# mitchelldurbincs/GeneralsReinforcementLearning

Hardware: AMD Instinct MI355X
Metric: env steps/sec (whole node), 20x20 4P fog-on; state bit-exact vs the C restatement of the Go engine (the reference's own test vectors pass on both) (higher is better)
Workload: dtype int32

## Files before the change

### generalsreinforcementlearning_amd/_lib.py

```python
import ctypes as C
import os

_PKG = os.path.dirname(os.path.abspath(__file__))
_LIB = None


class GvecError(RuntimeError):
    def __init__(self, code, msg):
        super().__init__(f"gvec error {code}: {msg}")
        self.code = code


class Config(C.Structure):
    _fields_ = [("abi_version", C.c_int32), ("num_envs", C.c_int32), ("max_width", C.c_int32), ("max_height", C.c_int32),
                ("max_players", C.c_int32), ("device", C.c_int32), ("fog_of_war", C.c_int32), ("prod_general", C.c_int32),
                ("prod_city", C.c_int32), ("prod_normal", C.c_int32), ("normal_growth_interval", C.c_int32),
                ("auto_reset", C.c_int32), ("reserved", C.c_int32 * 4)]


STATE_FIELDS = ["army", "owner", "type", "visible", "listed", "changed", "vis_changed", "turn", "done", "winner", "width",
                "height", "players", "alive", "army_count", "tile_count", "general_idx"]


class StateView(C.Structure):
# ... 89 lines not shown
    "gvec_reset_generated": (_i32, [_vp, _u64, _vp, _vp, _vp]),
    "gvec_reset_go_seeded": (_i32, [_vp, _vp, _vp, _vp, _vp]),
    "gvec_build_board_pool": (_i32, [_vp, _i32, _u64, _vp, _vp, _vp]),
    "gvec_step": (_i32, [_vp, _vp, _vp, _vp, _i32]),
    "gvec_legal_mask": (_i32, [_vp, _vp, _i32]),
    "gvec_player_visibility": (_i32, [_vp, _i32, _vp, _vp, _i32]),
    "gvec_read_state": (_i32, [_vp, _i32, _i32, C.POINTER(StateView), _i32]),
    "gvec_write_state": (_i32, [_vp, _i32, _i32, C.POINTER(StateView), _i32]),
    "gvec_rollout": (_i32, [_vp, _i32, _u64, _i32, _i32, C.POINTER(RolloutStats)]),
    "gvec_rollout_range": (_i32, [_vp, _i32, _i32, _i32, _u64, _i32]),
    "gvec_set_agent_mix": (_i32, [_vp, _i32, _i32]),
    "gvec_agent_actions": (_i32, [_vp, _u64, _i32, _vp, _i32]),
    "gvec_bot_actions": (_i32, [_vp, C.c_uint32, _u64, _i32, _vp, _i32]),
    "gvec_counters": (_i32, [_vp, C.POINTER(RolloutStats)]),
    "gvec_step_traffic_bytes": (_i32, [_vp, C.POINTER(C.c_int64)]),
    "gvec_experience_begin": (_i32, [_vp]),
    "gvec_experience_begin_range": (_i32, [_vp, _i32, _i32]),
    "gvec_experience_rewards": (_i32, [_vp, _vp, _vp, _i32]),
    "gvec_experience_record_layout": (_i32, [_vp, C.POINTER(C.c_int32)]),
    "gvec_experience_record_bytes": (_i32, [_vp]),
    "gvec_experience_records": (_i32, [_vp, _vp, _i32, _i32, _i32, _i32, _vp]),
    "gvec_record_agent_actions": (_i32, [_vp, _i32]),
    "gvec_expand_experience_records": (_i32, [_i32, _vp, C.POINTER(C.c_int32), _vp, _i32, _vp, _vp, _vp, _vp]),
    "gvec_pool_collect": (_i32, [_i32, _vp, C.POINTER(CollectArgs)]),
    "gvec_pool_collect_scratch_bytes": (_u64, [_i32]),
    "gvec_per_tree_bytes": (_u64, [C.c_int64]),
    "gvec_per_tree_layout": (_i32, [C.c_int64, C.POINTER(C.c_int64)]),
    "gvec_per_init": (_i32, [_i32, _vp, _vp, C.c_int64]),
    "gvec_per_push": (_i32, [_i32, _vp, _vp, C.c_int64, _vp, _vp, C.c_int64]),
    "gvec_per_update": (_i32, [_i32, _vp, _vp, C.c_int64, _vp, _vp, C.c_int64, C.c_float, C.c_float]),
# ... 67 lines not shown
```

### generalsreinforcementlearning_amd/csrc/gvec_api.hip

```cpp
#include <cstdarg>
#include <cstdio>
#include <new>

#include "gvec_handle.hpp"

static thread_local char g_err[512] = "";
void set_err(const char* fmt, ...) {
  va_list ap;
  va_start(ap, fmt);
  vsnprintf(g_err, sizeof g_err, fmt, ap);
  va_end(ap);
}

int32_t DevBuf::in_stage() const {
  if (slot >= 0) return GVEC_OK;
  set_err("a call staged more than %d arguments through its handle", Stage::kSlots);
  return GVEC_E_INVALID;
}

hipError_t DevBuf::alloc(size_t bytes) {
  if (bytes < 16) bytes = 16;
  if (h->stage_cap[slot] < bytes) {
    if (h->stage_ptr[slot]) {
      hipError_t e = hipStreamSynchronize(h->stream);
// ... 143 lines not shown
  h->stride = cfg->max_width * cfg->max_height;
  h->maxp = cfg->max_players;
  if (!pick_variant(cfg->max_players, h->stride, &h->var)) {
    set_err("no kernel variant for %d players / %d tiles", cfg->max_players, h->stride);
    return false;
  }
  h->fd = (h->stride <= 32 * (2 * h->var.nslot - 1)) ? 2 * h->var.nslot - 1 : 2 * h->var.nslot;
  h->row_dw = (int)round_up((size_t)(3 * h->var.maxp + 13) * h->fd, 4);
  h->army_dw = h->var.nslot * 64;
  h->mask_bytes = 16 * h->fd;
  h->mask_dw = h->mask_bytes / 4;
  h->stream = nullptr;
  return true;
}

extern "C" {

int32_t gvec_abi_version(void) { return GVEC_ABI_VERSION; }
const char* gvec_last_error(void) { return g_err; }

int32_t gvec_config_default(gvec_config* cfg) {
  if (!cfg) return GVEC_E_INVALID;
  memset(cfg, 0, sizeof *cfg);
  cfg->abi_version = GVEC_ABI_VERSION;
  cfg->num_envs = 1;
  cfg->max_width = 20;
  cfg->max_height = 20;
  cfg->max_players = 2;
  cfg->device = 0;
  cfg->fog_of_war = 1;
// ... 168 lines not shown
  return GVEC_OK;
}
int32_t gvec_host_free(void* p) {
  if (!p) return GVEC_OK;
  HIPCHK(hipHostFree(p));
  return GVEC_OK;
}

int32_t gvec_num_envs(const gvec_handle* h) { return h ? h->cfg.num_envs : GVEC_E_INVALID; }
int32_t gvec_tile_stride(const gvec_handle* h) { return h ? h->stride : GVEC_E_INVALID; }
int32_t gvec_mask_bytes(const gvec_handle* h) { return h ? h->mask_bytes : GVEC_E_INVALID; }
int64_t gvec_state_bytes_per_env(const gvec_handle* h) {
  return h ? (int64_t)4 * (HDR_DW + h->row_dw + h->army_dw) : (int64_t)GVEC_E_INVALID;
}

int32_t gvec_read_buffer(gvec_handle* h, int32_t which, uint64_t byte_offset, uint64_t bytes, void* host_dst) {
  if (!h || !host_dst) return GVEC_E_INVALID;
  if (h->sharded()) return sharded::unsupported("gvec_read_buffer");
  const size_t B = (size_t)h->cfg.num_envs;
  size_t total = 0;
  const void* base = nullptr;
  switch (which) {
    case GVEC_BUF_HEADER: base = h->d_hdr; total = B * HDR_DW * 4; break;
    case GVEC_BUF_LEGAL: base = h->d_legal; total = B * h->maxp * h->mask_bytes; break;
    case GVEC_BUF_ACTIONS: base = h->d_actions; total = B * h->maxp * sizeof(gvec_action); break;
    case GVEC_BUF_ERR: base = h->d_err; total = B * 4; break;
    default:
      set_err("gvec_read_buffer: buffer %d is not one of header / legal masks / actions / err", which);
      return GVEC_E_INVALID;
  }
// ... 43 lines not shown
```

### generalsreinforcementlearning_amd/csrc/gvec_api_engine.hip

```cpp
#include "gvec_handle.hpp"

namespace sharded {

static int32_t reset(gvec_handle* h, const int32_t* env_ids, int32_t n, const int32_t* army, const int8_t* owner, const uint8_t* type,
                     const int32_t* width, const int32_t* height, const int32_t* players, int32_t mem) {
  RET_IF(host_only(mem, "gvec_reset"));
  const size_t st = (size_t)h->stride;
  if (!env_ids) {
    return fan_range(h, 0, n, [=](gvec_handle* c, int lb, int cnt, size_t skip) {
      return gvec_reset(c, nullptr, cnt, army + skip * st, owner + skip * st, type + skip * st, width + skip, height + skip, players + skip, GVEC_MEM_HOST);
    });
  }
  struct Part {
    std::vector<int32_t> ids, w, hh, p, army;
    std::vector<int8_t> owner;
    std::vector<uint8_t> type;
  };
  auto parts = std::make_shared<std::vector<Part>>(h->shards.size());
  for (int i = 0; i < n; ++i) {
    const int e = env_ids[i];
    if (e < 0 || e >= h->cfg.num_envs) return GVEC_E_RANGE;
    size_t k = 0;
    while (e >= h->shards[k]->begin + h->shards[k]->n) ++k;
    Part& P = (*parts)[k];
// ... 325 lines not shown
  HIPCHK(hipSetDevice(h->cfg.device));
  HIPCHK(hipMemsetAsync(h->d_counters, 0, 3 * sizeof(unsigned long long), h->stream));
  HIPCHK(launch_counter_sum(h->d_hdr, h->cfg.num_envs, h->d_counters, h->stream));
  unsigned long long c[3];
  HIPCHK(hipMemcpyAsync(c, h->d_counters, sizeof c, hipMemcpyDeviceToHost, h->stream));
  HIPCHK(hipStreamSynchronize(h->stream));
  out->env_steps = (int64_t)c[0];
  out->aborted_turns = (int64_t)c[1];
  out->games_finished = (int64_t)c[2];
  out->reserved = 0;
  return GVEC_OK;
}

int32_t gvec_step_traffic_bytes(const gvec_handle* h, int64_t* out4) {
  if (!h || !out4) return GVEC_E_INVALID;
  static_assert(Planes<4>::MUTABLE == 2 * 4 + 3 && Planes<4>::LST - Planes<4>::MUTABLE == 10 && Planes<4>::COUNT - Planes<4>::LST == 4,
                "gvec_step_traffic_bytes restates the plane block's partition");
  const int64_t fd = h->fd, mp = h->var.maxp;
  const int nslot = h->var.nslot;
  const bool odd = fd == 2 * nslot - 1;
  const int64_t hdr = HDR_DW * 4;
  const int64_t mut = (2 * mp + 3) * fd * 4;
  const int64_t cst = (lean_derive_ok(nslot) ? 6 : 10) * fd * 4;
  const int64_t lst = mp * fd * 4;
  const int64_t a16 = (int64_t)h->army_dw * 2, a32 = (int64_t)h->army_dw * 4;
  out4[0] = hdr + mut + cst + a16 - (lean_half_last(nslot, odd) ? 64 : 0);
  out4[1] = hdr + mut + lean_fold_dwords((int)(2 * mp + 3), (int)fd) * 4 + a16;
  out4[2] = (int64_t)h->maxp * h->mask_bytes;
  out4[3] = 2 * lst + 2 * a32;
  return GVEC_OK;
}

int32_t gvec_agent_actions(gvec_handle* h, uint64_t seed, int32_t invalid_permille, gvec_action* actions, int32_t mem) {
  if (!h || !actions) return GVEC_E_INVALID;
  if (h->sharded()) {
    const size_t mp = (size_t)h->maxp;
    return sharded::fan_host(h, mem, "gvec_agent_actions", [=](gvec_handle* c, int begin, int) {
      return gvec_agent_actions(c, seed, invalid_permille, actions + begin * mp, GVEC_MEM_HOST);
    });
  }
  HIPCHK(hipSetDevice(h->cfg.device));
  StepArgs a = base_args(h);
  set_agent_seed(&a, seed, invalid_permille);
  a.actions_out = (mem == GVEC_MEM_HOST) ? h->d_actions : actions;
// ... 44 lines not shown
```

### generalsreinforcementlearning_amd/csrc/gvec_device.hpp

```cpp
#pragma once
#include <hip/hip_runtime.h>
#include <stdint.h>

#include "../../include/generals_vec.h"

extern "C" __device__ int gvec_llvm_writelane(int value, int lane, int vdst_in) __asm("llvm.amdgcn.writelane.i32");

#ifndef GVEC_NT
#define GVEC_NT 14
#endif
#define GVEC_NT_MASK 2
#define GVEC_NT_PLANE 4
#define GVEC_NT_ARMY 8
#ifndef GVEC_SC1
#define GVEC_SC1 1
#endif

#ifndef GVEC_LEAN
#define GVEC_LEAN 7
#endif

namespace gvec {

constexpr bool lean_derive_ok(int nslot) { return (GVEC_LEAN & 1) != 0 && 2 * nslot < 64 / (nslot <= 7 ? 4 : 2); }
constexpr bool lean_half_last(int nslot, bool odd) { return (GVEC_LEAN & 2) != 0 && odd && (nslot & 1) != 0; }
constexpr int lean_fold_dwords(int mutable_planes, int fd) { return (GVEC_LEAN & 4) != 0 ? ((mutable_planes * fd + 3) & ~3) - mutable_planes * fd : 0; }

typedef uint32_t u32x4 __attribute__((ext_vector_type(4)));

template <typename T>
__device__ __forceinline__ T ld_stream(const T* p) {
  if constexpr ((GVEC_NT & 1) != 0) return __builtin_nontemporal_load(p);
  return *p;
}
__device__ __forceinline__ void st_through(uint32_t* p, uint32_t v) { asm volatile("global_store_dword %0, %1, off sc1 nt" : : "v"(p), "v"(v) : "memory"); }
__device__ __forceinline__ void st_through(uint16_t* p, uint16_t v) {
  asm volatile("global_store_short %0, %1, off sc1 nt" : : "v"(p), "v"((uint32_t)v) : "memory");
}
__device__ __forceinline__ void st_through(float* p, float v) { asm volatile("global_store_dword %0, %1, off sc1 nt" : : "v"(p), "v"(v) : "memory"); }
__device__ __forceinline__ void st_through(u32x4* p, u32x4 v) {
  asm volatile("global_store_dwordx4 %0, %1, off sc1 nt\n\ts_nop 1" : : "v"(p), "v"(v) : "memory");
// ... 18 lines not shown
  H_GIDX = 12,
  H_RECIPW = 20,
  H_CNT_STEPS = 21,
  H_CNT_ABORT = 22,
  H_CNT_DONE = 23
};
constexpr uint32_t HF_DONE = 1u, HF_FOG = 2u, HF_WIDE = 4u;
constexpr uint32_t HF_SETUP = 8u;
constexpr uint32_t HF_SYNC = 16u;
constexpr uint32_t HF_VSMALL = 32u;
constexpr uint32_t HF_LDIFF = 128u;
constexpr uint32_t HF_FEWSPECIAL = 64u;

template <int MAXP>
struct Planes {
  static constexpr int OWN = 0, VIS = MAXP, CHG = 2 * MAXP, VCH = 2 * MAXP + 1, GT1 = 2 * MAXP + 2,
                       GEN = 2 * MAXP + 3, CITY = 2 * MAXP + 4, MTN = 2 * MAXP + 5, VALID = 2 * MAXP + 6, NCOL0 = 2 * MAXP + 7,
                       NCOLL = 2 * MAXP + 8, OK = 2 * MAXP + 9 , LST = 2 * MAXP + 13,
                       COUNT = 3 * MAXP + 13, MUTABLE = 2 * MAXP + 3, SHARED = 13 ;
};

constexpr uint32_t KF_AGENT = 1u;
constexpr uint32_t KF_EMIT = 2u;
constexpr uint32_t KF_AUTORESET = 4u;
constexpr uint32_t KF_LMVALID = 16u;

struct StepArgs {
  uint32_t* hdr;
  uint32_t* rows;
  uint32_t* army16;
  int32_t* army32;
  const gvec_action* actions;
  gvec_action* actions_out;
  int32_t* err;
// ... 323 lines not shown
```

### generalsreinforcementlearning_amd/csrc/gvec_kernels.hip

```cpp
#include "gvec_dispatch.hpp"
#include "gvec_turn.hpp"

namespace gvec {

constexpr int step_waves(int maxp, int nslot) {
  const int ppr = (nslot <= 7) ? 4 : 2;
  const int nr = (maxp + ppr - 1) / ppr;
  const int state = 3 * nr + 13 + nr + nslot + 4 * nr;
  const int need = state + (state + 32 <= 62 ? 32 : 40);
  const int alloc = (need + 7) / 8 * 8;
  const int w = 512 / alloc;
  return w > 8 ? 8 : (w < 2 ? 2 : w);
}

template <int MAXP, int NSLOT, bool AGENT, bool ODD>
__global__ __launch_bounds__(64 * WAVES_PER_BLOCK, step_waves(MAXP, NSLOT)) void step_kernel(StepArgs A) {
  constexpr int FD = 2 * NSLOT - (ODD ? 1 : 0);
  constexpr int ROW_DW = (Planes<MAXP>::COUNT * FD + 3) / 4 * 4;
  __shared__ int32_t army_shadow[WAVES_PER_BLOCK][NSLOT * 64];
  using B = Turn<MAXP, NSLOT>;
  __shared__ uint32_t act_scratch[WAVES_PER_BLOCK][B::ACT_SCRATCH_DW];
  const int wave = (int)(threadIdx.x >> 6), lane = lane_id();
  const int env = uni((int)blockIdx.x * WAVES_PER_BLOCK + wave);
  if (env >= A.num_envs) return;
  bool force_redeal = false;
  if constexpr (!AGENT) {
    const uint32_t f0 = (uint32_t)uni((int)reinterpret_cast<const uint32_t*>(A.actions)[((size_t)env * A.pstride) * 2 + 1]);
    if (f0 & GVEC_ACT_SKIP_ENV) {
      if (A.err && lane == 0) A.err[env] = 0;
      return;
    }
    force_redeal = (f0 & GVEC_ACT_RESET_ENV) != 0u;
  }
  B b;
  b.larmy = army_shadow[wave];
  b.lscr = act_scratch[wave];
  const ArmyRef army_env = army_ref<NSLOT>(A.army16, A.army32, env);
  load_turn<true, lean_half_last(NSLOT, ODD)>(b, A.hdr + (size_t)env * HDR_DW, A.rows + (size_t)env * ROW_DW, army_env, FD, A.zeros);
  b.small = !(b.hflags & HF_WIDE);
  const bool emit = (A.flags & KF_EMIT) != 0u;
  uint32_t m[B::NR][4];
  uint32_t err = 0u;
  bool types_dirty = false, changed = true;
  const bool can_redeal = (A.flags & KF_AUTORESET) && A.pool_size > 0;
  if (AGENT && A.actions_out && (b.hflags & HF_DONE)) {
    if (lane < A.pstride) reinterpret_cast<uint2*>(A.actions_out)[(size_t)env * A.pstride + lane] = make_uint2(0u, 0u);
  }
  if (can_redeal && ((b.hflags & HF_DONE) || force_redeal)) {
    redeal<MAXP, NSLOT>(b, A, env, FD, ROW_DW);
    types_dirty = true;
  } else if (b.hflags & HF_DONE) {
    err = GVEC_ERR_GAME_OVER;
    changed = false;
// ... 14 lines not shown
      if (A.actions_out) {
        uint32_t alo, ahi;
        agent_words<MAXP, NSLOT>(b, mine, alo, ahi);
        if (lane < A.pstride) reinterpret_cast<uint2*>(A.actions_out)[(size_t)env * A.pstride + lane] = make_uint2(alo, ahi);
      }
    } else {
      uint32_t alo = 0u, ahi = 0u;
      if (lane < A.pstride) {
        const uint2 w = reinterpret_cast<const uint2*>(A.actions)[(size_t)env * A.pstride + lane];
        alo = w.x;
        ahi = w.y;
      }
      av = b.prevalidate(alo, ahi);
    }
    bool aborted;
    err = b.turn_step(av, A, aborted);
    if (!(GVEC_PROFILE_SKIP & 32)) b.refresh_gt1();
    if (GVEC_PROFILE_DUP & 32) { b.opaque_v(); b.refresh_gt1(); }
    b.hdr_set(H_CNT_STEPS, b.hdr_get(H_CNT_STEPS) + 1u);
    if (aborted) b.hdr_set(H_CNT_ABORT, b.hdr_get(H_CNT_ABORT) + 1u);
    if (b.hflags & HF_DONE) b.hdr_set(H_CNT_DONE, b.hdr_get(H_CNT_DONE) + 1u);
  }
  b.store_army_staged(army_env);
  b.settle_lists();
  b.store_hdr(A.hdr + (size_t)env * HDR_DW, err);
  if (types_dirty) b.store_planes(A.rows + (size_t)env * ROW_DW, FD, ROW_DW, true);
  else b.store_planes_staged(A.rows + (size_t)env * ROW_DW, FD);
  if (A.err && lane == 0) A.err[env] = (int32_t)err;
  if (!(GVEC_PROFILE_SKIP & 64) && emit && (changed || !(A.flags & KF_LMVALID))) {
    b.template legal_planes<false>(m);
    b.store_masks_staged(m, A.legal + (size_t)env * A.pstride * A.mask_dw, FD, A.pstride);
// ... 398 lines not shown
```

### generalsreinforcementlearning_amd/csrc/gvec_packed.hpp

```cpp
#pragma once
#include "gvec_device.hpp"

#ifndef GVEC_PROFILE_SKIP
#define GVEC_PROFILE_SKIP 0
#endif
#ifndef GVEC_PROFILE_DUP
#define GVEC_PROFILE_DUP 0
#endif
#ifndef GVEC_ACT_VECTOR
#define GVEC_ACT_VECTOR 1
#endif

namespace gvec {

template <int ROWL>
__device__ __forceinline__ uint32_t row_scan_add(uint32_t v) {
  v += dpp0<0x111>(v);
  v += dpp0<0x112>(v);
  v += dpp0<0x114>(v);
  v += dpp0<0x118>(v);
  if constexpr (ROWL == 32) v += dpp0<0x142, 0xa>(v);
  return v;
}
template <int ROWL>
// ... 52 lines not shown
  static_assert(!(DERIVE_OK && FULL_ROWS), "lean_derive_ok leaves the full-row variants alone");
  static constexpr int NPACKED = DERIVE_OK ? PL::OK - PL::CHG : NSHARED;
  static constexpr int NSR = (NPACKED + PPR - 1) / PPR;
  uint32_t shp[NSR];
  int32_t army[NSLOT];
  uint32_t hv;
  int32_t* larmy;
  uint32_t* lscr = nullptr;
  int W, H, P, N, turn, recipW;
  uint32_t alive, hflags;
  bool small = false;
  int32_t move_delta = 0;
  uint32_t prod_mask = 0u;
  int32_t prod_rate = 0;
  bool prod_uniform = false, grow = false;

  static __device__ __forceinline__ int col() { return lane_id() & (ROWL - 1); }
  static __device__ __forceinline__ int row() { return lane_id() / ROWL; }
  static __device__ __forceinline__ int lane_player(int k) { return k * PPR + row(); }
  __device__ __forceinline__ bool lane_flag(uint32_t bits, int k) const { return (bits & rowbit[k]) != 0u; }
  static __device__ __forceinline__ bool in_row_of(int p) { return row() == (p % PPR); }

  static __device__ __forceinline__ uint32_t prev_lane(uint32_t m) {
    const uint32_t v = from_prev(m);
    if constexpr (FULL_ROWS) return (col() == 0) ? 0u : v;
    return v;
  }
  static __device__ __forceinline__ uint32_t next_lane(uint32_t m) {
    const uint32_t v = from_next(m);
    if constexpr (FULL_ROWS) return (col() == ROWL - 1) ? 0u : v;
// ... 40 lines not shown
    W = (int)(dims & 0xFFu);
    H = (int)((dims >> 8) & 0xFFu);
    P = (int)((dims >> 16) & 0xFFu);
    hflags = dims >> 24;
    N = W * H;
    alive = k[H_STATUS] & 0xFFu;
    recipW = (int)k[H_RECIPW];
  }
  __device__ __forceinline__ void land_scalars() {
    asm volatile("" : "+s"(turn), "+s"(W), "+s"(H), "+s"(P), "+s"(hflags), "+s"(alive), "+s"(recipW));
  }
  __device__ __forceinline__ void load_hdr(const uint32_t* hdr_env) {
    issue_hdr(hdr_env);
    decode_hdr();
  }
  __device__ __forceinline__ void land() {
    asm volatile("" : "+v"(hv));
#pragma unroll
    for (int k = 0; k < NR; ++k) {
      asm volatile("" : "+v"(own[k]));
      asm volatile("" : "+v"(lst[k]));
      asm volatile("" : "+v"(vis[k]));
    }
#pragma unroll
    for (int k = 0; k < NSR; ++k) asm volatile("" : "+v"(shp[k]));
  }
  __device__ __forceinline__ void opaque() {
    opaque_v();
    asm volatile("" : "+s"(turn), "+s"(alive), "+s"(hflags));
  }
  __device__ __forceinline__ void opaque_v() {
    asm volatile("" : "+v"(hv));
#pragma unroll
    for (int s = 0; s < NSLOT; ++s) asm volatile("" : "+v"(army[s]));
#pragma unroll
    for (int k = 0; k < NR; ++k) {
      asm volatile("" : "+v"(own[k]));
// ... 1 lines not shown
      asm volatile("" : "+v"(vis[k]));
    }
    asm volatile("" : "+v"(chg));
    asm volatile("" : "+v"(vch));
    asm volatile("" : "+v"(gt1));
  }
  __device__ __forceinline__ void hdr_set(int k, uint32_t v) { hv = (uint32_t)gvec_llvm_writelane((int)v, k, (int)hv); }
  __device__ __forceinline__ uint32_t hdr_get(int k) const { return rdlane(hv, k); }
  __device__ __forceinline__ void store_hdr(uint32_t* hdr_env, uint32_t last_err) {
    hdr_set(H_TURN, (uint32_t)turn);
    hdr_set(H_DIMS, (uint32_t)W | ((uint32_t)H << 8) | ((uint32_t)P << 16) | (hflags << 24));
    hdr_set(H_STATUS, alive | (last_err << 16));
    if (lane_id() < HDR_DW) st_stream<GVEC_NT_PLANE>(hdr_env + lane_id(), hv);
  }

  template <bool PACK = true>
  __device__ __forceinline__ void load_planes(const uint32_t* rows_env, int fd, const uint32_t* zeros) {
    const bool in = col() < fd;
    const uint32_t* lane_base = rows_env + (row() * fd + col());
    if constexpr (PACK) {
#pragma unroll
      for (int k = 0; k < NR; ++k) {
        own[k] = vis[k] = 0u;
        if (in && (k * PPR + row() < MAXP)) {
          own[k] = ld_stream(lane_base + (PL::OWN + k * PPR) * fd);
          vis[k] = ld_stream(lane_base + (PL::VIS + k * PPR) * fd);
        }
      }
#pragma unroll
      for (int k = 0; k < NSR; ++k) {
        shp[k] = 0u;
        if (in && (k * PPR + row() < NPACKED)) shp[k] = ld_stream(lane_base + (PL::CHG + k * PPR) * fd);
      }
    } else {
#pragma unroll
      for (int k = 0; k < NR; ++k) {
        const uint32_t* gp = (in && (k * PPR + row() < MAXP)) ? lane_base : zeros;
        own[k] = ld_stream(gp + (PL::OWN + k * PPR) * fd);
        vis[k] = ld_stream(gp + (PL::VIS + k * PPR) * fd);
      }
      load_lists(rows_env, fd);
      const uint32_t* gs = in ? rows_env + col() : zeros;
      chg = ld_stream(gs + PL::CHG * fd);
      vch = ld_stream(gs + PL::VCH * fd);
      gt1 = ld_stream(gs + PL::GT1 * fd);
      gen = ld_stream(gs + PL::GEN * fd);
      city = ld_stream(gs + PL::CITY * fd);
      mtn = ld_stream(gs + PL::MTN * fd);
      valid = ld_stream(gs + PL::VALID * fd);
      ncol0 = ld_stream(gs + PL::NCOL0 * fd);
      ncolL = ld_stream(gs + PL::NCOLL * fd);
#pragma unroll
      for (int d = 0; d < 4; ++d) ok[d] = ld_stream(gs + (PL::OK + d) * fd);
    }
  }
  __device__ __forceinline__ void load_lists(const uint32_t* rows_env, int fd) {
#pragma unroll
    for (int k = 0; k < NR; ++k) lst[k] = own[k];
    if (hflags & HF_LDIFF) {
      const uint32_t* lane_base = rows_env + (row() * fd + col());
#pragma unroll
      for (int k = 0; k < NR; ++k) {
        lst[k] = 0u;
        if (col() < fd && (k * PPR + row() < MAXP)) lst[k] = lane_base[(PL::LST + k * PPR) * fd];
      }
    }
  }
  __device__ __forceinline__ void settle_lists() { hflags = lists_match() ? (hflags & ~HF_LDIFF) : (hflags | HF_LDIFF); }
// ... 53 lines not shown
        g[PL::VALID * fd] = valid;
        g[PL::NCOL0 * fd] = ncol0;
        g[PL::NCOLL * fd] = ncolL;
#pragma unroll
        for (int d = 0; d < 4; ++d) g[(PL::OK + d) * fd] = ok[d];
      }
    }
    if (with_types && lane < row_dw - PL::COUNT * fd) rows_env[PL::COUNT * fd + lane] = 0u;
  }
  __device__ __forceinline__ void load_army(const ArmyCRef& a) {
    army_load_narrow<NSLOT>(army, a.n);
    if (hflags & HF_WIDE) army_load_wide<NSLOT>(army, a.w);
  }
  template <bool HALF_LAST = false>
  __device__ __forceinline__ void load_army_narrow(const ArmyCRef& a) { army_load_narrow<NSLOT, HALF_LAST>(army, a.n); }
  __device__ __forceinline__ void load_army_wide_if_flagged(const ArmyCRef& a) {
    if (hflags & HF_WIDE) army_load_wide<NSLOT>(army, a.w);
  }
  __device__ __forceinline__ void store_army(const ArmyRef& a) {
    if (army_fits_narrow<NSLOT>(army)) {
      hflags &= ~HF_WIDE;
      army_store_narrow<NSLOT>(army, a.n);
    } else {
      hflags |= HF_WIDE;
      army_store_wide<NSLOT>(army, a.w);
    }
  }

  __device__ __forceinline__ void army_to_lds() {
#pragma unroll
    for (int s = 0; s < NSLOT; ++s) larmy[64 * s + lane_id()] = army[s];
    wave_lds_fence();
// ... 39 lines not shown
#pragma unroll
    for (int k = 0; k < NR; ++k) d |= lst[k] ^ own[k];
    return !any_bit(d);
  }
  __device__ __forceinline__ void refresh_gt1() {
    uint32_t g = 0u;
#pragma unroll
    for (int s = 0; s < NSLOT; ++s) {
      const unsigned long long b = __builtin_amdgcn_ballot_w64(army[s] > 1);
      g = (uint32_t)gvec_llvm_writelane((int)(uint32_t)b, 2 * s, (int)g);
      g = (uint32_t)gvec_llvm_writelane((int)(uint32_t)(b >> 32), 2 * s + 1, (int)g);
    }
    gt1 = replicate_row0(g);
  }

  __device__ __forceinline__ void update_fog(bool matched = false) {
    if (!(hflags & HF_FOG)) return;
    bool full, none;
    if ((hflags & HF_VSMALL) && turn > 0 && P <= N / 10) {
      full = false;
      none = !any_bit(vch);
    } else {
      const int nv = count_shared(vch);
      full = turn == 0 || nv > N / 10;
      none = nv == 0;
    }
    if (full) {
#pragma unroll
      for (int k = 0; k < NR; ++k) {
        const uint32_t d = dil3(lst[k]);
        vis[k] = lane_flag(alive, k) ? d : 0u;
      }
      return;
    }
    if (none) return;
    const uint32_t near3 = dil3(vch), clr = ~near3;
    const uint32_t near5 = matched ? 0u : dil3(near3);
#pragma unroll
    for (int k = 0; k < NR; ++k) {
      const uint32_t d = dil3(lst[k]);
      const unsigned long long hit = __builtin_amdgcn_ballot_w64((matched ? (d & near3) : (own[k] & near5)) != 0u);
      const uint32_t mine = (uint32_t)(hit >> (row() * ROWL)) & (ROWL == 32 ? 0xFFFFFFFFu : 0xFFFFu);
      const bool relit = mine != 0u && lane_flag(alive, k);
      vis[k] = (vis[k] & clr) | (relit ? d : 0u);
    }
  }

  __device__ __forceinline__ uint32_t multi_sum(const int32_t (&acc)[MAXP]) const {
    static_assert(MAXP == 2 || MAXP == 4 || MAXP == 8, "fold levels are written for 2, 4 or 8 players");
    static_assert(H_ARMYCNT == 4, "the final row_shl assumes header lanes 4..4+MAXP-1");
    const int lane = lane_id();
    uint32_t m[MAXP];
#pragma unroll
    for (int p = 0; p < MAXP; ++p) m[p] = (uint32_t)acc[p];
    {
      const bool hi = (lane & 1) != 0;
#pragma unroll
      for (int i = 0; i < MAXP / 2; ++i) {
        const uint32_t keep = hi ? m[2 * i + 1] : m[2 * i], give = hi ? m[2 * i] : m[2 * i + 1];
// ... 312 lines not shown
      for (int k = 0; k < NR; ++k) {
        own[k] = (lane_player(k) == v) ? (own[k] & ~tiles) : own[k];
        own[k] = (lane_player(k) == nw) ? (own[k] | tiles) : own[k];
      }
      hdr_set(H_GIDX + v, 0xFFFFFFFFu);
      chg |= tiles;
      vch |= tiles;
      hflags &= ~HF_VSMALL;
      alive &= ~(1u << v);
    }
  }

  __device__ __forceinline__ uint32_t turn_step(uint32_t acts_lo, uint32_t acts_hi, const StepArgs& A, bool& aborted) {
    return turn_step(prevalidate(acts_lo, acts_hi), A, aborted);
  }
  __device__ __forceinline__ uint32_t turn_step(const ActVec& av, const StepArgs& A, bool& aborted) {
    aborted = false;
    turn++;
    const bool matched = lists_match();
    if (!(GVEC_PROFILE_SKIP & 2)) update_fog(matched);
    if (GVEC_PROFILE_DUP & 2) { opaque(); update_fog(matched); }
    chg = 0u;
    vch = 0u;
    hflags |= HF_VSMALL;
    bool delta = matched && (hflags & HF_SYNC) != 0u;
    move_delta = 0;
    uint32_t first_err = 0u, elim_seen = 0u;
    uint64_t orders = 0ull;
    int n_orders = 0;
    const unsigned long long present = __builtin_amdgcn_ballot_w64((av.meta & 16u) != 0u && lane_id() < P);
    if (present && !(GVEC_PROFILE_SKIP & 4)) {
      army_to_lds();
      if (!(GVEC_ACT_VECTOR && lscr && act_vector(av, first_err, orders, n_orders, elim_seen))) {
        act_chain<0>(av, first_err, orders, n_orders, elim_seen);
        delta = false;
      }
// ... 57 lines not shown
    u32x4* g4 = reinterpret_cast<u32x4*>(dst);
    const int chunks = dwords >> 2;
    for (int i = lane_id(); i < chunks; i += 64) {
      st_stream<CLASS>(g4 + i, s4[i]);
    }
    const int tail = dwords & 3, l = lane_id();
    if (l < tail) st_stream<CLASS>(dst + 4 * chunks + l, reinterpret_cast<const uint32_t*>(larmy)[4 * chunks + l]);
  }
  __device__ __forceinline__ void store_planes_staged(uint32_t* rows_env, int fd) const {
    uint32_t* stage = reinterpret_cast<uint32_t*>(larmy);
    const bool in = col() < fd;
    uint32_t* g = stage + row() * fd + col();
    wave_lds_fence();
#pragma unroll
    for (int k = 0; k < NR; ++k) {
      if (in && (k * PPR + row() < MAXP)) {
        g[(PL::OWN + k * PPR) * fd] = own[k];
        g[(PL::VIS + k * PPR) * fd] = vis[k];
      }
    }
#pragma unroll
    for (int k = 0; k * PPR < 3; ++k) {
      const int j = k * PPR + row();
      if (in && j < 3) g[(PL::CHG + k * PPR) * fd] = j == 0 ? chg : (j == 1 ? vch : gt1);
    }
    const int gap = lean_fold_dwords(PL::MUTABLE, fd);
    if (in && row() == 0) {
      if (col() < gap) g[PL::GEN * fd] = gen;
      if (fd + col() < gap) g[PL::CITY * fd] = city;
      if (2 * fd + col() < gap) g[PL::MTN * fd] = mtn;
    }
    wave_lds_fence();
    flush_stage<GVEC_NT_PLANE>(rows_env, PL::MUTABLE * fd + gap);
    store_lists(rows_env, fd);
  }
  __device__ __forceinline__ void store_army_narrow_staged(uint32_t* n) const {
    uint32_t* stage = reinterpret_cast<uint32_t*>(larmy);
    const int lane = lane_id();
    wave_lds_fence();
#pragma unroll
    for (int k = 0; k < NSLOT / 2; ++k) stage[64 * k + lane] = (uint32_t)army[2 * k] | ((uint32_t)army[2 * k + 1] << 16);
    if constexpr ((NSLOT & 1) != 0) reinterpret_cast<uint16_t*>(stage + 64 * (NSLOT / 2))[lane] = (uint16_t)army[NSLOT - 1];
    wave_lds_fence();
    flush_stage<GVEC_NT_ARMY>(n, NSLOT * 32);
  }
  __device__ __forceinline__ void store_army_staged(const ArmyRef& a) {
    if (army_fits_narrow<NSLOT>(army)) {
      hflags &= ~HF_WIDE;
// ... 31 lines not shown
```

### generalsreinforcementlearning_amd/csrc/gvec_turn.hpp

```cpp
#pragma once
#include "gvec_launch.hpp"
#include "gvec_packed.hpp"

namespace gvec {

template <int MAXP, int NSLOT>
using Turn = PBoard<MAXP, NSLOT>;

template <int MAXP, int NSLOT>
__device__ __forceinline__ uint32_t agent_sample(const Turn<MAXP, NSLOT>& b, const uint32_t (&m)[Turn<MAXP, NSLOT>::NR][4], uint32_t ek,
                                                 const StepArgs& A) {
  using T = Turn<MAXP, NSLOT>;
  constexpr int NR = T::NR, PPR = T::PPR, ROWL = T::ROWL;
  const int lane = lane_id();
  const uint32_t sbase = ek + (uint32_t)b.turn * 0x9E3779B1u + 0x165667B1u;
  uint32_t mine = 0u;
#pragma unroll
  for (int k = 0; k < NR; ++k) {
    const uint32_t player = (uint32_t)T::lane_player(k);
    const uint32_t h1 = amix(mad24(player, 0x4A7C15u, sbase));
    const uint32_t h2 = amix(h1 ^ 0x68E31DA4u);
    const uint32_t hi16 = h2 >> 16;
    const bool act = b.lane_flag(b.alive, k) && !((h1 & 0xFFFFu) < A.agent_noop);
    const bool half = (h1 >> 16) < A.agent_half;
// ... 44 lines not shown
    const bool off = (d == 0) ? (y == 0) : (d == 1) ? (x == b.W - 1) : (d == 2) ? (y == b.H - 1) : (x == 0);
    code = off ? GVEC_ERR_INVALID_COORDINATES : 0u;
  }
  v.meta = act ? (code | 16u | ((mine & 0x2000u) ? 32u : 0u)) : 0u;
  v.ft = t;
  v.tt = t + ((d == 0) ? -b.W : (d == 1) ? 1 : (d == 2) ? b.W : -1);
  return v;
}

template <typename BT>
__device__ __forceinline__ void load_board(BT& b, const uint32_t* hdr, const uint32_t* rows, const ArmyCRef& army, int fd) {
  b.load_hdr(hdr);
  b.load_army(army);
  b.load_planes(rows, fd);
}
template <bool EARLY = false, bool HALF_LAST = false, typename BT>
__device__ __forceinline__ void load_turn(BT& b, const uint32_t* hdr, const uint32_t* rows, const ArmyCRef& army, int fd, const uint32_t* zeros) {
  if constexpr (EARLY) {
    b.issue_hdr(hdr);
    b.load_planes(rows, fd, zeros);
    b.template load_army_narrow<HALF_LAST>(army);
    b.decode_hdr_scalar(hdr);
    b.land();
    b.land_scalars();
    b.spread_shared();
    b.load_lists(rows, fd);
    b.load_army_wide_if_flagged(army);
  } else {
    b.load_hdr(hdr);
    b.load_army(army);
    b.template load_planes<false>(rows, fd, zeros);
  }
}

template <int MAXP, int NSLOT, typename BT>
__device__ __forceinline__ void redeal(BT& b, const StepArgs& A, int env, int fd, int row_dw) {
  const uint32_t episode = b.hdr_get(H_EPISODE) + 1u;
  const uint32_t cs = b.hdr_get(H_CNT_STEPS), ca = b.hdr_get(H_CNT_ABORT), cd = b.hdr_get(H_CNT_DONE);
  const uint32_t hk = fmix32(env_key_of(A.pool_seed_base, (uint32_t)env) ^ (episode * 0x9E3779B1u));
  const int j = (int)__umulhi(hk, (uint32_t)A.pool_size);
  load_turn(b, A.pool_hdr + (size_t)j * HDR_DW, A.pool_rows + (size_t)j * row_dw, army_cref<NSLOT>(A.pool_army16, A.pool_army32, j), fd, A.zeros);
  b.hdr_set(H_EPISODE, episode);
// ... 7 lines not shown
```

### generalsreinforcementlearning_amd/env_state.py

```python
import json

import numpy as np

from ._lib import GvecError
from .vec_engine import VecEngine

GVEC_E_INVALID, GVEC_E_RANGE = -1, -4
FORMAT_VERSION = 1
CONFIG_KEYS = ("board_width", "board_height", "max_players", "fog_of_war", "production", "normal_growth_interval", "max_turns",
               "learners")


class VecEnvState:

    def __init__(self, engine, env_ids, turn_count, resetting, stream, pool, config):
        self.engine, self.env_ids, self.turn_count, self.resetting = engine, env_ids, turn_count, resetting
        self.stream, self.pool, self.config = stream, pool, config

    @property
    def num_envs(self):
        return self.engine.B

    def save(self, path):
        import torch
# ... 157 lines not shown
```

### include/generals_vec.h

```cpp
#ifndef GENERALS_VEC_H
#define GENERALS_VEC_H

#include <stdint.h>

#ifdef __cplusplus
extern "C" {
#endif

#define GVEC_ABI_VERSION 2

#define GVEC_MAX_PLAYERS 8
#define GVEC_MAX_DIM     32

#define GVEC_OK            0
#define GVEC_E_INVALID    -1
#define GVEC_E_NO_DEVICE  -2
#define GVEC_E_HIP        -3
#define GVEC_E_RANGE      -4
#define GVEC_E_BOARD      -5

#define GVEC_ERR_NONE                 0
#define GVEC_ERR_INVALID_COORDINATES  1
#define GVEC_ERR_NOT_ADJACENT         2
#define GVEC_ERR_NOT_OWNED            3
// ... 110 lines not shown
int32_t gvec_player_visibility(gvec_handle* h, int32_t player,
                               uint8_t* visible, uint8_t* fog, int32_t mem);

int32_t gvec_read_state(gvec_handle* h, int32_t env_begin, int32_t n,
                        const gvec_state_view* view, int32_t mem);
int32_t gvec_write_state(gvec_handle* h, int32_t env_begin, int32_t n,
                         const gvec_state_view* view, int32_t mem);

int32_t gvec_rollout(gvec_handle* h, int32_t turns, uint64_t seed,
                     int32_t invalid_permille, int32_t fused,
                     gvec_rollout_stats* stats);
int32_t gvec_rollout_range(gvec_handle* h, int32_t env_begin, int32_t n, int32_t turns, uint64_t seed, int32_t invalid_permille);
int32_t gvec_set_agent_mix(gvec_handle* h, int32_t noop_per_65536, int32_t half_per_65536);
int32_t gvec_counters(gvec_handle* h, gvec_rollout_stats* out);
int32_t gvec_step_traffic_bytes(const gvec_handle* h, int64_t* out4);
int32_t gvec_agent_actions(gvec_handle* h, uint64_t seed, int32_t invalid_permille,
                           gvec_action* actions, int32_t mem);
int32_t gvec_bot_actions(gvec_handle* h, uint32_t players, uint64_t seed, int32_t random_permille,
                         gvec_action* actions, int32_t mem);

int32_t gvec_experience_begin(gvec_handle* h);
int32_t gvec_experience_begin_range(gvec_handle* h, int32_t env_begin, int32_t n);
int32_t gvec_experience_rewards(gvec_handle* h, float* rewards, uint8_t* done, int32_t mem);

int32_t gvec_experience_record_layout(gvec_handle* h, int32_t* out8);
int32_t gvec_experience_record_bytes(gvec_handle* h);
int32_t gvec_experience_records(gvec_handle* h, const gvec_action* actions, int32_t mem, int32_t env_begin,
                                int32_t n, int32_t env_id_base, void* dst_device);
int32_t gvec_expand_experience_records(int32_t device, void* hip_stream, const int32_t* layout8, const void* records, int32_t n,
                                       float* state, float* next_state, uint8_t* action_mask, int32_t* meta);
// ... 176 lines not shown
```

Before: 1.267 billion.

## Load and store visibility planes on demand instead of every turn

Moves the per-player visibility planes out of the mutable block in the per-env row layout so the per-turn load no longer reads them. Fog updates are deferred: lit masks are computed, visibility is loaded only when an incremental fog update is needed, and it is written back only when fog changed. This cuts per-step global memory traffic for fog-on boards in exchange for an extra conditional load/store path and a changed state layout (format version bumped). It also adds an API that reports the plane partition and the traffic estimate.

```diff
diff --git a/generalsreinforcementlearning_amd/_lib.py b/generalsreinforcementlearning_amd/_lib.py
--- a/generalsreinforcementlearning_amd/_lib.py
+++ b/generalsreinforcementlearning_amd/_lib.py
@@ -127,6 +127,7 @@
     "gvec_bot_actions": (_i32, [_vp, C.c_uint32, _u64, _i32, _vp, _i32]),
     "gvec_counters": (_i32, [_vp, C.POINTER(RolloutStats)]),
     "gvec_step_traffic_bytes": (_i32, [_vp, C.POINTER(C.c_int64)]),
+    "gvec_layout_partition": (_i32, [C.POINTER(Config), C.POINTER(C.c_int32), C.POINTER(C.c_int64)]),
     "gvec_experience_begin": (_i32, [_vp]),
     "gvec_experience_begin_range": (_i32, [_vp, _i32, _i32]),
     "gvec_experience_rewards": (_i32, [_vp, _vp, _vp, _i32]),
diff --git a/generalsreinforcementlearning_amd/csrc/gvec_api.hip b/generalsreinforcementlearning_amd/csrc/gvec_api.hip
--- a/generalsreinforcementlearning_amd/csrc/gvec_api.hip
+++ b/generalsreinforcementlearning_amd/csrc/gvec_api.hip
@@ -181,6 +181,16 @@
   return true;
 }
 
+template <int MAXP>
+static void plane_partition(int nslot, int fd, int32_t* o) {
+  using PL = Planes<MAXP>;
+  const int32_t v[] = {fd, (PL::COUNT * fd + 3) / 4 * 4, PL::OWN, PL::CHG, PL::GEN, PL::OK, PL::VIS, PL::LST, PL::COUNT, PL::MUTABLE,
+                       lean_derive_ok(nslot) ? 1 : 0, lean_half_last(nslot, fd == 2 * nslot - 1) ? 1 : 0, lean_fold_dwords(PL::MUTABLE, fd),
+                       lean_vis_on_demand() ? 1 : 0, HDR_DW, nslot * 64};
+  static_assert(sizeof v == 16 * sizeof(int32_t), "gvec_layout_partition fills 16 values");
+  memcpy(o, v, sizeof v);
+}
+
 extern "C" {
 
 int32_t gvec_abi_version(void) { return GVEC_ABI_VERSION; }
@@ -379,6 +389,17 @@
   return h ? (int64_t)4 * (HDR_DW + h->row_dw + h->army_dw) : (int64_t)GVEC_E_INVALID;
 }
 
+int32_t gvec_layout_partition(const gvec_config* cfg, int32_t* out16, int64_t* traffic4) {
+  if (!cfg || !out16 || !traffic4) return GVEC_E_INVALID;
+  gvec_handle h;
+  if (cfg->max_width < 1 || cfg->max_height < 1 || cfg->max_players < 1 || !set_geometry(&h, cfg)) return GVEC_E_INVALID;
+  if (h.var.maxp == 2) plane_partition<2>(h.var.nslot, h.fd, out16);
+  else if (h.var.maxp == 4) plane_partition<4>(h.var.nslot, h.fd, out16);
+  else plane_partition<8>(h.var.nslot, h.fd, out16);
+  if (out16[1] != h.row_dw) return GVEC_E_INVALID;
+  return gvec_step_traffic_bytes(&h, traffic4);
+}
+
 int32_t gvec_read_buffer(gvec_handle* h, int32_t which, uint64_t byte_offset, uint64_t bytes, void* host_dst) {
   if (!h || !host_dst) return GVEC_E_INVALID;
   if (h->sharded()) return sharded::unsupported("gvec_read_buffer");
diff --git a/generalsreinforcementlearning_amd/csrc/gvec_api_engine.hip b/generalsreinforcementlearning_amd/csrc/gvec_api_engine.hip
--- a/generalsreinforcementlearning_amd/csrc/gvec_api_engine.hip
+++ b/generalsreinforcementlearning_amd/csrc/gvec_api_engine.hip
@@ -363,20 +363,23 @@
 
 int32_t gvec_step_traffic_bytes(const gvec_handle* h, int64_t* out4) {
   if (!h || !out4) return GVEC_E_INVALID;
-  static_assert(Planes<4>::MUTABLE == 2 * 4 + 3 && Planes<4>::LST - Planes<4>::MUTABLE == 10 && Planes<4>::COUNT - Planes<4>::LST == 4,
+  static_assert(Planes<4>::MUTABLE == 4 + 3 && Planes<4>::VIS - Planes<4>::MUTABLE == 10 && Planes<4>::LST - Planes<4>::VIS == 4 &&
+                    Planes<4>::COUNT - Planes<4>::LST == 4,
                 "gvec_step_traffic_bytes restates the plane block's partition");
   const int64_t fd = h->fd, mp = h->var.maxp;
   const int nslot = h->var.nslot;
   const bool odd = fd == 2 * nslot - 1;
   const int64_t hdr = HDR_DW * 4;
-  const int64_t mut = (2 * mp + 3) * fd * 4;
+  const int64_t mut = (mp + 3) * fd * 4;
   const int64_t cst = (lean_derive_ok(nslot) ? 6 : 10) * fd * 4;
+  const int64_t vis = mp * fd * 4;
   const int64_t lst = mp * fd * 4;
   const int64_t a16 = (int64_t)h->army_dw * 2, a32 = (int64_t)h->army_dw * 4;
-  out4[0] = hdr + mut + cst + a16 - (lean_half_last(nslot, odd) ? 64 : 0);
-  out4[1] = hdr + mut + lean_fold_dwords((int)(2 * mp + 3), (int)fd) * 4 + a16;
+  const int64_t every = lean_vis_on_demand() ? 0 : vis;
+  out4[0] = hdr + mut + cst + every + a16 - (lean_half_last(nslot, odd) ? 64 : 0);
+  out4[1] = hdr + mut + every + lean_fold_dwords((int)(mp + 3), (int)fd) * 4 + a16;
   out4[2] = (int64_t)h->maxp * h->mask_bytes;
-  out4[3] = 2 * lst + 2 * a32;
+  out4[3] = 2 * (vis - every) + 2 * lst + 2 * a32;
   return GVEC_OK;
 }
 
diff --git a/generalsreinforcementlearning_amd/csrc/gvec_device.hpp b/generalsreinforcementlearning_amd/csrc/gvec_device.hpp
--- a/generalsreinforcementlearning_amd/csrc/gvec_device.hpp
+++ b/generalsreinforcementlearning_amd/csrc/gvec_device.hpp
@@ -17,7 +17,7 @@
 #endif
 
 #ifndef GVEC_LEAN
-#define GVEC_LEAN 7
+#define GVEC_LEAN 15
 #endif
 
 namespace gvec {
@@ -25,6 +25,7 @@
 constexpr bool lean_derive_ok(int nslot) { return (GVEC_LEAN & 1) != 0 && 2 * nslot < 64 / (nslot <= 7 ? 4 : 2); }
 constexpr bool lean_half_last(int nslot, bool odd) { return (GVEC_LEAN & 2) != 0 && odd && (nslot & 1) != 0; }
 constexpr int lean_fold_dwords(int mutable_planes, int fd) { return (GVEC_LEAN & 4) != 0 ? ((mutable_planes * fd + 3) & ~3) - mutable_planes * fd : 0; }
+constexpr bool lean_vis_on_demand() { return (GVEC_LEAN & 8) != 0; }
 
 typedef uint32_t u32x4 __attribute__((ext_vector_type(4)));
 
@@ -73,10 +74,10 @@
 
 template <int MAXP>
 struct Planes {
-  static constexpr int OWN = 0, VIS = MAXP, CHG = 2 * MAXP, VCH = 2 * MAXP + 1, GT1 = 2 * MAXP + 2,
-                       GEN = 2 * MAXP + 3, CITY = 2 * MAXP + 4, MTN = 2 * MAXP + 5, VALID = 2 * MAXP + 6, NCOL0 = 2 * MAXP + 7,
-                       NCOLL = 2 * MAXP + 8, OK = 2 * MAXP + 9 , LST = 2 * MAXP + 13,
-                       COUNT = 3 * MAXP + 13, MUTABLE = 2 * MAXP + 3, SHARED = 13 ;
+  static constexpr int OWN = 0, CHG = MAXP, VCH = MAXP + 1, GT1 = MAXP + 2, GEN = MAXP + 3, CITY = MAXP + 4, MTN = MAXP + 5,
+                       VALID = MAXP + 6, NCOL0 = MAXP + 7, NCOLL = MAXP + 8, OK = MAXP + 9 ,
+                       VIS = MAXP + 13, LST = 2 * MAXP + 13, COUNT = 3 * MAXP + 13, MUTABLE = MAXP + 3,
+                       SHARED = 13 ;
 };
 
 constexpr uint32_t KF_AGENT = 1u;
diff --git a/generalsreinforcementlearning_amd/csrc/gvec_kernels.hip b/generalsreinforcementlearning_amd/csrc/gvec_kernels.hip
--- a/generalsreinforcementlearning_amd/csrc/gvec_kernels.hip
+++ b/generalsreinforcementlearning_amd/csrc/gvec_kernels.hip
@@ -36,7 +36,8 @@
   b.larmy = army_shadow[wave];
   b.lscr = act_scratch[wave];
   const ArmyRef army_env = army_ref<NSLOT>(A.army16, A.army32, env);
-  load_turn<true, lean_half_last(NSLOT, ODD)>(b, A.hdr + (size_t)env * HDR_DW, A.rows + (size_t)env * ROW_DW, army_env, FD, A.zeros);
+  constexpr bool LEAN_VIS = lean_vis_on_demand();
+  load_turn<true, lean_half_last(NSLOT, ODD), LEAN_VIS>(b, A.hdr + (size_t)env * HDR_DW, A.rows + (size_t)env * ROW_DW, army_env, FD, A.zeros);
   b.small = !(b.hflags & HF_WIDE);
   const bool emit = (A.flags & KF_EMIT) != 0u;
   uint32_t m[B::NR][4];
@@ -81,7 +82,8 @@
       av = b.prevalidate(alo, ahi);
     }
     bool aborted;
-    err = b.turn_step(av, A, aborted);
+    err = b.template turn_step<LEAN_VIS>(av, A, aborted, A.rows + (size_t)env * ROW_DW, FD);
+    if constexpr (LEAN_VIS) b.apply_fog();
     if (!(GVEC_PROFILE_SKIP & 32)) b.refresh_gt1();
     if (GVEC_PROFILE_DUP & 32) { b.opaque_v(); b.refresh_gt1(); }
     b.hdr_set(H_CNT_STEPS, b.hdr_get(H_CNT_STEPS) + 1u);
diff --git a/generalsreinforcementlearning_amd/csrc/gvec_packed.hpp b/generalsreinforcementlearning_amd/csrc/gvec_packed.hpp
--- a/generalsreinforcementlearning_amd/csrc/gvec_packed.hpp
+++ b/generalsreinforcementlearning_amd/csrc/gvec_packed.hpp
@@ -90,6 +90,8 @@
   uint32_t prod_mask = 0u;
   int32_t prod_rate = 0;
   bool prod_uniform = false, grow = false;
+  int fog_mode = 0;
+  uint32_t fog_clr = 0u, fog_lit[NR];
 
   static __device__ __forceinline__ int col() { return lane_id() & (ROWL - 1); }
   static __device__ __forceinline__ int row() { return lane_id() / ROWL; }
@@ -160,13 +162,14 @@
     issue_hdr(hdr_env);
     decode_hdr();
   }
+  template <bool LEAN_VIS = false>
   __device__ __forceinline__ void land() {
     asm volatile("" : "+v"(hv));
 #pragma unroll
     for (int k = 0; k < NR; ++k) {
       asm volatile("" : "+v"(own[k]));
       asm volatile("" : "+v"(lst[k]));
-      asm volatile("" : "+v"(vis[k]));
+      if constexpr (!LEAN_VIS) asm volatile("" : "+v"(vis[k]));
     }
 #pragma unroll
     for (int k = 0; k < NSR; ++k) asm volatile("" : "+v"(shp[k]));
@@ -198,8 +201,9 @@
     if (lane_id() < HDR_DW) st_stream<GVEC_NT_PLANE>(hdr_env + lane_id(), hv);
   }
 
-  template <bool PACK = true>
+  template <bool PACK = true, bool LEAN_VIS = false>
   __device__ __forceinline__ void load_planes(const uint32_t* rows_env, int fd, const uint32_t* zeros) {
+    static_assert(PACK || !LEAN_VIS, "only the per-turn load leaves the visibility planes out");
     const bool in = col() < fd;
     const uint32_t* lane_base = rows_env + (row() * fd + col());
     if constexpr (PACK) {
@@ -208,7 +212,7 @@
         own[k] = vis[k] = 0u;
         if (in && (k * PPR + row() < MAXP)) {
           own[k] = ld_stream(lane_base + (PL::OWN + k * PPR) * fd);
-          vis[k] = ld_stream(lane_base + (PL::VIS + k * PPR) * fd);
+          if constexpr (!LEAN_VIS) vis[k] = ld_stream(lane_base + (PL::VIS + k * PPR) * fd);
         }
       }
 #pragma unroll
@@ -236,6 +240,14 @@
       ncolL = ld_stream(gs + PL::NCOLL * fd);
 #pragma unroll
       for (int d = 0; d < 4; ++d) ok[d] = ld_stream(gs + (PL::OK + d) * fd);
+    }
+  }
+  __device__ __forceinline__ void load_vis(const uint32_t* rows_env, int fd) {
+    const uint32_t* lane_base = rows_env + (row() * fd + col());
+#pragma unroll
+    for (int k = 0; k < NR; ++k) {
+      vis[k] = 0u;
+      if (col() < fd && (k * PPR + row() < MAXP)) vis[k] = ld_stream(lane_base + (PL::VIS + k * PPR) * fd);
     }
   }
   __device__ __forceinline__ void load_lists(const uint32_t* rows_env, int fd) {
@@ -319,8 +331,15 @@
   }
   template <bool HALF_LAST = false>
   __device__ __forceinline__ void load_army_narrow(const ArmyCRef& a) { army_load_narrow<NSLOT, HALF_LAST>(army, a.n); }
+  template <bool LAND = false>
   __device__ __forceinline__ void load_army_wide_if_flagged(const ArmyCRef& a) {
-    if (hflags & HF_WIDE) army_load_wide<NSLOT>(army, a.w);
+    if (hflags & HF_WIDE) {
+      army_load_wide<NSLOT>(army, a.w);
+      if constexpr (LAND) {
+#pragma unroll
+        for (int s = 0; s < NSLOT; ++s) asm volatile("" : "+v"(army[s]));
+      }
+    }
   }
   __device__ __forceinline__ void store_army(const ArmyRef& a) {
     if (army_fits_narrow<NSLOT>(army)) {
@@ -390,7 +409,9 @@
     gt1 = replicate_row0(g);
   }
 
-  __device__ __forceinline__ void update_fog(bool matched = false) {
+  template <bool DEFER = false>
+  __device__ __forceinline__ void update_fog(bool matched = false, const uint32_t* rows_env = nullptr, int fd = 0) {
+    fog_mode = 0;
     if (!(hflags & HF_FOG)) return;
     bool full, none;
     if ((hflags & HF_VSMALL) && turn > 0 && P <= N / 10) {
@@ -405,11 +426,15 @@
 #pragma unroll
       for (int k = 0; k < NR; ++k) {
         const uint32_t d = dil3(lst[k]);
-        vis[k] = lane_flag(alive, k) ? d : 0u;
-      }
+        const uint32_t lit = lane_flag(alive, k) ? d : 0u;
+        if constexpr (DEFER) fog_lit[k] = lit;
+        else vis[k] = lit;
+      }
+      fog_mode = 2;
       return;
     }
     if (none) return;
+    if constexpr (DEFER) load_vis(rows_env, fd);
     const uint32_t near3 = dil3(vch), clr = ~near3;
     const uint32_t near5 = matched ? 0u : dil3(near3);
 #pragma unroll
@@ -418,7 +443,19 @@
       const unsigned long long hit = __builtin_amdgcn_ballot_w64((matched ? (d & near3) : (own[k] & near5)) != 0u);
       const uint32_t mine = (uint32_t)(hit >> (row() * ROWL)) & (ROWL == 32 ? 0xFFFFFFFFu : 0xFFFFu);
       const bool relit = mine != 0u && lane_flag(alive, k);
-      vis[k] = (vis[k] & clr) | (relit ? d : 0u);
+      if constexpr (DEFER) fog_lit[k] = relit ? d : 0u;
+      else vis[k] = (vis[k] & clr) | (relit ? d : 0u);
+    }
+    fog_clr = clr;
+    fog_mode = 1;
+  }
+  __device__ __forceinline__ void apply_fog() {
+    if (fog_mode == 1) {
+#pragma unroll
+      for (int k = 0; k < NR; ++k) vis[k] = (vis[k] & fog_clr) | fog_lit[k];
+    } else if (fog_mode == 2) {
+#pragma unroll
+      for (int k = 0; k < NR; ++k) vis[k] = fog_lit[k];
     }
   }
 
@@ -761,12 +798,13 @@
   __device__ __forceinline__ uint32_t turn_step(uint32_t acts_lo, uint32_t acts_hi, const StepArgs& A, bool& aborted) {
     return turn_step(prevalidate(acts_lo, acts_hi), A, aborted);
   }
-  __device__ __forceinline__ uint32_t turn_step(const ActVec& av, const StepArgs& A, bool& aborted) {
+  template <bool DEFER_VIS = false>
+  __device__ __forceinline__ uint32_t turn_step(const ActVec& av, const StepArgs& A, bool& aborted, const uint32_t* rows_env = nullptr, int fd = 0) {
     aborted = false;
     turn++;
     const bool matched = lists_match();
-    if (!(GVEC_PROFILE_SKIP & 2)) update_fog(matched);
-    if (GVEC_PROFILE_DUP & 2) { opaque(); update_fog(matched); }
+    if (!(GVEC_PROFILE_SKIP & 2)) update_fog<DEFER_VIS>(matched, rows_env, fd);
+    if (GVEC_PROFILE_DUP & 2) { opaque(); update_fog<DEFER_VIS>(matched, rows_env, fd); }
     chg = 0u;
     vch = 0u;
     hflags |= HF_VSMALL;
@@ -854,16 +892,14 @@
     wave_lds_fence();
 #pragma unroll
     for (int k = 0; k < NR; ++k) {
-      if (in && (k * PPR + row() < MAXP)) {
-        g[(PL::OWN + k * PPR) * fd] = own[k];
-        g[(PL::VIS + k * PPR) * fd] = vis[k];
-      }
+      if (in && (k * PPR + row() < MAXP)) g[(PL::OWN + k * PPR) * fd] = own[k];
     }
 #pragma unroll
     for (int k = 0; k * PPR < 3; ++k) {
       const int j = k * PPR + row();
       if (in && j < 3) g[(PL::CHG + k * PPR) * fd] = j == 0 ? chg : (j == 1 ? vch : gt1);
     }
+    static_assert(PL::GEN == PL::MUTABLE && PL::CITY == PL::GEN + 1 && PL::MTN == PL::GEN + 2, "the fold reaches into GEN, CITY, MTN");
     const int gap = lean_fold_dwords(PL::MUTABLE, fd);
     if (in && row() == 0) {
       if (col() < gap) g[PL::GEN * fd] = gen;
@@ -872,6 +908,12 @@
     }
     wave_lds_fence();
     flush_stage<GVEC_NT_PLANE>(rows_env, PL::MUTABLE * fd + gap);
+    if (fog_mode != 0) {
+      uint32_t* gp = rows_env + row() * fd + col();
+#pragma unroll
+      for (int k = 0; k < NR; ++k)
+        if (in && (k * PPR + row() < MAXP)) st_stream<GVEC_NT_PLANE>(gp + (PL::VIS + k * PPR) * fd, vis[k]);
+    }
     store_lists(rows_env, fd);
   }
   __device__ __forceinline__ void store_army_narrow_staged(uint32_t* n) const {
diff --git a/generalsreinforcementlearning_amd/csrc/gvec_turn.hpp b/generalsreinforcementlearning_amd/csrc/gvec_turn.hpp
--- a/generalsreinforcementlearning_amd/csrc/gvec_turn.hpp
+++ b/generalsreinforcementlearning_amd/csrc/gvec_turn.hpp
@@ -82,18 +82,19 @@
   b.load_army(army);
   b.load_planes(rows, fd);
 }
-template <bool EARLY = false, bool HALF_LAST = false, typename BT>
+template <bool EARLY = false, bool HALF_LAST = false, bool LEAN_VIS = false, typename BT>
 __device__ __forceinline__ void load_turn(BT& b, const uint32_t* hdr, const uint32_t* rows, const ArmyCRef& army, int fd, const uint32_t* zeros) {
+  static_assert(EARLY || !LEAN_VIS, "only the per-turn load leaves the visibility planes out");
   if constexpr (EARLY) {
     b.issue_hdr(hdr);
-    b.load_planes(rows, fd, zeros);
+    b.template load_planes<true, LEAN_VIS>(rows, fd, zeros);
     b.template load_army_narrow<HALF_LAST>(army);
     b.decode_hdr_scalar(hdr);
-    b.land();
+    b.template land<LEAN_VIS>();
     b.land_scalars();
     b.spread_shared();
     b.load_lists(rows, fd);
-    b.load_army_wide_if_flagged(army);
+    b.template load_army_wide_if_flagged<LEAN_VIS>(army);
   } else {
     b.load_hdr(hdr);
     b.load_army(army);
diff --git a/generalsreinforcementlearning_amd/env_state.py b/generalsreinforcementlearning_amd/env_state.py
--- a/generalsreinforcementlearning_amd/env_state.py
+++ b/generalsreinforcementlearning_amd/env_state.py
@@ -6,7 +6,7 @@
 from .vec_engine import VecEngine
 
 GVEC_E_INVALID, GVEC_E_RANGE = -1, -4
-FORMAT_VERSION = 1
+FORMAT_VERSION = 2
 CONFIG_KEYS = ("board_width", "board_height", "max_players", "fog_of_war", "production", "normal_growth_interval", "max_turns",
                "learners")
 
diff --git a/include/generals_vec.h b/include/generals_vec.h
--- a/include/generals_vec.h
+++ b/include/generals_vec.h
@@ -148,6 +148,7 @@
 int32_t gvec_set_agent_mix(gvec_handle* h, int32_t noop_per_65536, int32_t half_per_65536);
 int32_t gvec_counters(gvec_handle* h, gvec_rollout_stats* out);
 int32_t gvec_step_traffic_bytes(const gvec_handle* h, int64_t* out4);
+int32_t gvec_layout_partition(const gvec_config* cfg, int32_t* out16, int64_t* traffic4);
 int32_t gvec_agent_actions(gvec_handle* h, uint64_t seed, int32_t invalid_permille,
                            gvec_action* actions, int32_t mem);
 int32_t gvec_bot_actions(gvec_handle* h, uint32_t players, uint64_t seed, int32_t random_permille,
```

After: 1.171 billion. 7.6% lower.
